# clawrim/gcn10

Hardware: AMD Instinct MI355X
Metric: CN Gpixels/sec (higher is better)
Workload: dtype u8

## Files before the change

### gcn10_amd/csrc/gcn10_context.hip

```cpp

#include <hip/hip_runtime.h>
#include <unistd.h>
#include <hip/hip_ext.h>

#include <cstdarg>
#include <cstdint>
#include <cstdio>
#include <cstring>
#include <new>

#include "gcn10_gpu.h"
#include "gcn10_device_util.hpp"
#include "gcn10_gpu_internal.hpp"
#include "gcn10_soil_readers.hpp"

using gcn10::as_stream;
using gcn10::fail;
using gcn10::kLut16Bytes;
using gcn10::kLut1Bytes;
using gcn10::use_device;

namespace gcn10 {

thread_local char g_err[512] = "";
// ... 430 lines not shown
            continue;
        ctx->opt.*o.field = value;
        if (o.field == &gcn10_gpu_ctx::Options::ilp1)
            ctx->opt.single.set = false;
        return GCN10_OK;
    }
    return fail(GCN10_E_INVAL, "gcn10_gpu_set_option: unknown option or bad value: %s=%d", name, value);
}

int gcn10_gpu_time_next_strip(gcn10_gpu_ctx *ctx, gcn10_event_t start, gcn10_event_t stop)
{
    if (!ctx || !start || !stop)
        return fail(GCN10_E_INVAL, "gcn10_gpu_time_next_strip: null argument");
    ctx->time_start = reinterpret_cast<hipEvent_t>(start);
    ctx->time_stop = reinterpret_cast<hipEvent_t>(stop);
    return GCN10_OK;
}

const char *gcn10_gpu_last_kernel_name(gcn10_gpu_ctx *ctx)
{
    return ctx ? ctx->last_kernel : "";
}

}
```

### gcn10_amd/csrc/gcn10_gpu_internal.hpp

```cpp
#ifndef GCN10_GPU_INTERNAL_HPP
#define GCN10_GPU_INTERNAL_HPP

#include <hip/hip_runtime.h>

#include <cstdint>

#include "gcn10_gpu.h"
#include "gcn10_strip_lanes.hpp"

namespace gcn10 {

int fail(int code, const char *fmt, ...) __attribute__((format(printf, 2, 3)));

#define HIP_TRY(expr)                                                                   \
    do {                                                                                \
        hipError_t e_ = (expr);                                                         \
        if (e_ != hipSuccess)                                                           \
            return gcn10::fail(e_ == hipErrorOutOfMemory ? GCN10_E_NOMEM : GCN10_E_HIP, \
                               "%s: %s", #expr, hipGetErrorString(e_));                 \
    } while (0)

int use_device(gcn10_gpu_ctx *ctx);
hipStream_t as_stream(gcn10_gpu_ctx *ctx, gcn10_stream_t s);
int grow_workspace(void **ws, size_t *cap, size_t need);
// ... 61 lines not shown

    struct SingleShape {
        bool set = false;
        int xcd_slabs = 1, grid_blocks_per_cu = 8, ilp = 2, prefetch = 1;
    };

    struct Options {
        int grid_blocks_per_cu = 16;
        int ilp16 = 0;
        int ilp1 = 2;
        int nontemporal = 1;
        int xcd_slabs = 1;
        int prefetch = 1;
        int compact_soil = 1;
        SingleShape single;
        int arena_segment_align = 4096;
        int deflate_wave_codes = 1;
        int fused_parse = 1;
        int fused_emit = 1;
        int event_sync_sleep_us = 0;
    } opt;

    const char *last_kernel = "";
    hipEvent_t time_start = nullptr, time_stop = nullptr;
    bool fused_ready = false;
    bool codes_ready = false;
    bool deflate_ready = false;

    struct Workspaces {
        void *deflate = nullptr;
        size_t deflate_cap = 0;
        void *inflate = nullptr;
        size_t inflate_cap = 0;
        void *lzw = nullptr;
        size_t lzw_cap = 0;
    } ws;
};

#endif
```

### gcn10_amd/csrc/gcn10_soil_readers.hpp

```cpp
#ifndef GCN10_SOIL_READERS_HPP
#define GCN10_SOIL_READERS_HPP

#include "gcn10_gpu_internal.hpp"

namespace gcn10 {

struct SoilView {
    const uint8_t *hx;
    const int32_t *cj;
    uint32_t stride, rows;

    __device__ __forceinline__ uint32_t clamp(uint32_t r) const { return r < rows ? r : rows - 1u; }
    __device__ __forceinline__ uint32_t row(uint32_t y) const { return clamp((uint32_t)cj[y]); }
    __device__ __forceinline__ const uint8_t *at(uint32_t r, uint32_t x) const { return hx + (size_t)r * stride + x; }
    __device__ __forceinline__ const uint8_t *ptr(uint32_t y, uint32_t x) const { return at(row(y), x); }
};

constexpr int kPlanes = 6;
constexpr int kLut16Plane = 256 * 16 + 16;
constexpr int kLut16Bytes = kPlanes * kLut16Plane;
constexpr int kPlane1 = 256 + 4;
constexpr int kLut1Bytes = kPlanes * kPlane1;

template <int THREADS>
__device__ __forceinline__ void stage_lut16(uint8_t *lds, const uint8_t *src)
{
    for (int i = threadIdx.x; i < kLut16Bytes / 16; i += THREADS)
        reinterpret_cast<u32x4 *>(lds)[i] = reinterpret_cast<const u32x4 *>(src)[i];
}

__device__ __forceinline__ const uint8_t *lut16_row(const uint8_t *lut, uint32_t plane, uint32_t lc)
{
    return lut + plane * (uint32_t)kLut16Plane + lc * 16u;
}

__device__ __forceinline__ uint32_t lut16_value(const uint8_t *lut, uint32_t plane, uint32_t lc, uint32_t k)
{
    return lut16_row(lut, plane, lc)[k];
}

__device__ __forceinline__ uint32_t perm(uint32_t hi, uint32_t lo, uint32_t sel)
{
    return __builtin_amdgcn_perm(hi, lo, sel);
}

__device__ __forceinline__ void transpose4x4(uint32_t a, uint32_t b, uint32_t c, uint32_t d, uint32_t &o0,
                                             uint32_t &o1, uint32_t &o2, uint32_t &o3)
{
    const uint32_t t0 = perm(b, a, 0x05010400u);
    const uint32_t t1 = perm(b, a, 0x07030602u);
    const uint32_t t2 = perm(d, c, 0x05010400u);
// ... 42 lines not shown
```

### gcn10_amd/csrc/gcn10_strip.hip

```cpp

#include <hip/hip_runtime.h>

#include <cstdint>
#include <cstdio>
#include <cstring>

#include "gcn10_gpu.h"
#include "gcn10_device_util.hpp"
#include "gcn10_gpu_internal.hpp"
#include "gcn10_soil_readers.hpp"

using gcn10::aligned16;
using gcn10::as_stream;
using gcn10::fail;
using gcn10::first_chunk;
using gcn10::kChunk;
using gcn10::kLut16Bytes;
using gcn10::kLut1Bytes;
using gcn10::kPlane1;
using gcn10::kPxPerLane;
using gcn10::kThreads;
using gcn10::launch_timed;
using gcn10::load16_aligned;
using gcn10::load16_aligned_nt;
using gcn10::load16_any;
using gcn10::popcount;
using gcn10::scalar_load_i32;
using gcn10::SoilView;
// ... 14 lines not shown
    uint32_t npix;
    uint32_t nvec16;
    uint32_t nchunks;
    uint32_t table_mask;
    uint32_t single_k;
    uint32_t xcd_slabs;
    const uint32_t *cx;
    const uint8_t *codes;
    uint32_t codes_stride;
    const uint32_t *soil_complex;
    uint32_t soil_gen;
};

enum { kLut16 = 0, kLut1 = 1 };
constexpr uint32_t kWavePx = 64u * kPxPerLane;
constexpr uint32_t kMinVectorW = kWavePx + 16u;

enum { kSoilBytes = 0, kSoilLanes = 1, kSoilPixels = 2 };

template <int ILP>
struct Trip {
    u32x4 e16[ILP], c16[ILP];
    uint32_t i0[ILP];
};

template <int ILP, bool NT>
__device__ __forceinline__ void issue_trip(const StripParams &p, uint32_t trip, uint32_t lane_off,
                                           uint32_t wave_off, Trip<ILP> &tr)
{
    uint32_t xb[ILP], r0[ILP], r1[ILP], wb[ILP];
#pragma unroll
    for (int u = 0; u < ILP; u++) {
        wb[u] = __builtin_amdgcn_readfirstlane((trip * ILP + u) * (uint32_t)kChunk + wave_off);
        const uint32_t wbc = wb[u] < p.npix ? wb[u] : 0u;
        const uint32_t y = wbc / p.W;
        xb[u] = wbc - y * p.W;
        r0[u] = (uint32_t)scalar_load_i32(p.soil.cj, y);
        r1[u] = (uint32_t)scalar_load_i32(p.soil.cj, y + 1u < p.rows ? y + 1u : y);
    }
#pragma unroll
    for (int u = 0; u < ILP; u++) {
        tr.i0[u] = wb[u] + lane_off;
        const uint8_t *pe = p.esa + (tr.i0[u] < p.nvec16 ? tr.i0[u] : 0u);
        tr.e16[u] = NT ? load16_aligned_nt(pe) : load16_aligned(pe);
    }
#pragma unroll
    for (int u = 0; u < ILP; u++) {
        uint32_t xl = xb[u] + lane_off;
        const bool wrap = xl >= p.W;
        xl = wrap ? xl - p.W : xl;
        const uint32_t row = p.soil.clamp(wrap ? r1[u] : r0[u]);
        const uint8_t *pa = p.soil.at(row, xl);
        u32x4 a = load16_any(pa);
        if (p.W & 15u) {
            const uint32_t n = p.W - xl;
            const bool strad = !wrap && n < (uint32_t)kPxPerLane;
            if (__builtin_amdgcn_ballot_w64(strad) != 0ull) {
                const uint8_t *pb = strad ? p.soil.at(p.soil.clamp(r1[u]), 0u) - n : pa;
                const u32x4 b = load16_any(pb);
                const uint32_t nn = strad ? n : (uint32_t)kPxPerLane;
#pragma unroll
                for (int j = 0; j < 4; j++) {
                    const int32_t m = (int32_t)nn - 4 * j;
                    const uint32_t mask = m >= 4 ? 0xffffffffu : (m <= 0 ? 0u : (1u << (8 * m)) - 1u);
                    a[j] = (a[j] & mask) | (b[j] & ~mask);
                }
// ... 40 lines not shown
    if (SOIL == kSoilLanes) {
        uint32_t cx[16];
#pragma unroll
        for (int j = 0; j < 4; j++) {
            const u32x4 c4 = *reinterpret_cast<const u32x4 *>(p.cx + ls.x + 4 * j);
#pragma unroll
            for (int q = 0; q < 4; q++)
                cx[4 * j + q] = c4[q];
        }
        ls.c_lo = cx[0];
        ls.c_hi = cx[15];
        uint32_t split = 0;
#pragma unroll
        for (int q = 0; q < 16; q++)
            split += cx[q] == ls.c_lo && split == (uint32_t)q ? 1u : 0u;
        ls.split = (int32_t)split;
#pragma unroll
        for (int j = 0; j < 4; j++)
            ls.mask[j] = split_mask(ls.split, j);
        ls.pair = __builtin_amdgcn_ballot_w64(ls.c_hi - ls.c_lo > 1u) == 0ull;
    }
}

template <int ILP, bool NT, int SOIL>
__device__ __forceinline__ void issue_lane_trip(const StripParams &p, const LaneSoil &ls, uint32_t trip,
                                                Trip<ILP> &tr)
{
    uint32_t o0[ILP], o1[ILP];
#pragma unroll
    for (int u = 0; u < ILP; u++) {
        const uint32_t y = ls.y_first + (trip * ILP + u) * ls.B;
        const uint32_t ya = y < p.rows ? y : p.rows - 1u;
        const uint32_t yb = y + 1u < p.rows ? y + 1u : p.rows - 1u;
        o0[u] = p.soil.clamp((uint32_t)scalar_load_i32(p.soil.cj, ya)) * p.codes_stride;
        o1[u] = p.soil.clamp((uint32_t)scalar_load_i32(p.soil.cj, yb)) * p.codes_stride;
    }
#pragma unroll
    for (int u = 0; u < ILP; u++) {
        const uint32_t i0 = ls.base + (trip * ILP + u) * ls.sub_px;
        const bool live = i0 < ls.lim;
        tr.i0[u] = live ? i0 : 0xffffffffu;
        const uint8_t *pe = p.esa + (live ? i0 : 0u);
        tr.e16[u] = NT ? load16_aligned_nt(pe) : load16_aligned(pe);
    }
#pragma unroll
    for (int u = 0; u < ILP; u++) {
        const uint32_t off = ls.wrap ? o1[u] : o0[u];
        if (SOIL == kSoilLanes) {
            typedef uint16_t u16_u __attribute__((aligned(1)));
            tr.c16[u][0] = *reinterpret_cast<const u16_u *>(p.codes + (off + ls.c_lo));
            if (!ls.pair)
                tr.c16[u][1] = p.codes[off + ls.c_hi];
        }
        else {
            const uint8_t *cr = p.codes + off;
            const u32x4 *pc = reinterpret_cast<const u32x4 *>(p.cx + ls.x);
            u32x4 a = { 0u, 0u, 0u, 0u };
#pragma unroll 1
            for (int j = 0; j < 4; j++) {
                const u32x4 c4 = pc[j];
                const uint32_t w = (uint32_t)cr[c4[0]] | (uint32_t)cr[c4[1]] << 8 | (uint32_t)cr[c4[2]] << 16 |
                                   (uint32_t)cr[c4[3]] << 24;
                a[0] = j == 0 ? w : a[0];
                a[1] = j == 1 ? w : a[1];
                a[2] = j == 2 ? w : a[2];
                a[3] = j == 3 ? w : a[3];
            }
            tr.c16[u] = a;
        }
    }
}

template <bool KEEP_MASKS>
__device__ __forceinline__ u32x4 mix_lane_codes(const LaneSoil &ls, const u32x4 &c)
{
    const uint32_t a = (c[0] & 0xffu) * 0x01010101u;
    const uint32_t b = (ls.pair ? (c[0] >> 8) & 0xffu : c[1] & 0xffu) * 0x01010101u;
    u32x4 cd;
    int32_t split = ls.split;
    if (!KEEP_MASKS)
        asm volatile("" : "+v"(split));
#pragma unroll
    for (int j = 0; j < 4; j++) {
        const uint32_t mask = KEEP_MASKS ? ls.mask[j] : split_mask(split, j);
        cd[j] = (a & mask) | (b & ~mask);
    }
    return cd;
}

template <int KIND, int COND_MASK, int ILP, bool NT, int SOIL>
__device__ __forceinline__ void finish_trip(const StripParams &p, const uint8_t *lut, uint32_t tmask,
                                            const Trip<ILP> &tr, const LaneSoil &ls)
{
#pragma unroll
    for (int u = 0; u < ILP; u++) {
        const bool live = tr.i0[u] < p.nvec16;
        const u32x4 c16 = SOIL == kSoilLanes ? mix_lane_codes<KIND == kLut1>(ls, tr.c16[u]) : tr.c16[u];
#pragma unroll
        for (int c = 0; c < 2; c++) {
            if (!(COND_MASK & (1 << c)))
                continue;
            if (KIND == kLut16) {
                uint32_t acc[9][4];
                gcn10::gather16(lut, tr.e16[u], c16, c, acc);
                if (live) {
#pragma unroll
                    for (int k = 0; k < 9; k++) {
                        if (tmask & (1u << k)) {
                            u32x4 v = {acc[k][0], acc[k][1], acc[k][2], acc[k][3]};
                            store16<NT>(p.out[c * 9 + k] + tr.i0[u], v);
                        }
                    }
                }
            }
            else {
                u32x4 v;
#pragma unroll
                for (int j = 0; j < 4; j++) {
                    const uint32_t e = tr.e16[u][j];
                    const uint32_t cd = c16[j];
                    uint32_t w = 0;
#pragma unroll
                    for (int q = 0; q < 4; q++) {
                        const uint32_t lc = (e >> (8 * q)) & 0xffu;
                        const uint32_t s = (cd >> (8 * q + 4 * c)) & 0xfu;
                        const uint32_t b = lut[s * (uint32_t)kPlane1 + lc];
                        w |= b << (8 * q);
                    }
                    v[j] = w;
                }
                if (live)
                    store16<NT>(p.out[c * 9 + p.single_k] + tr.i0[u], v);
            }
        }
    }
}

template <int KIND, int COND_MASK, int ILP, bool NT, bool PF, int SOIL>
__device__ __forceinline__ void strip_loop(const StripParams &p, const uint8_t *lut, uint32_t tmask)
{
    uint32_t step = 1u, end, trip = 0u, lane_off = 0u, wave_off = 0u;
    LaneSoil ls = {};
    if (SOIL == kSoilBytes) {
        lane_off = (threadIdx.x & 63u) * kPxPerLane;
        wave_off = __builtin_amdgcn_readfirstlane(threadIdx.x >> 6) * kWavePx;
        trip = first_chunk(p.nchunks, step, end, p.xcd_slabs != 0);
    }
    else {
        const gcn10::StripLanePlan pl = gcn10::strip_lane_plan(p.W, p.rows, gridDim.x, blockIdx.x, threadIdx.x,
                                                               p.xcd_slabs != 0, (uint32_t)ILP);
        end = __builtin_amdgcn_readfirstlane(pl.trips);
        if (!__builtin_amdgcn_readfirstlane((uint32_t)pl.active))
            return;
        lane_prologue<SOIL>(p, pl, ls);
    }
    if (trip >= end)
        return;
    auto issue = [&](uint32_t t, Trip<ILP> &tr) {
        if (SOIL == kSoilBytes)
            issue_trip<ILP, NT>(p, t, lane_off, wave_off, tr);
        else
            issue_lane_trip<ILP, NT, SOIL>(p, ls, t, tr);
    };
    if (!PF) {
        for (; trip < end; trip += step) {
            Trip<ILP> tr;
            issue(trip, tr);
            finish_trip<KIND, COND_MASK, ILP, NT, SOIL>(p, lut, tmask, tr, ls);
        }
    }
    else {
        Trip<ILP> ta, tb;
        issue(trip, ta);
        for (;;) {
            trip += step;
            if (trip >= end) {
                finish_trip<KIND, COND_MASK, ILP, NT, SOIL>(p, lut, tmask, ta, ls);
                break;
            }
            issue(trip, tb);
            finish_trip<KIND, COND_MASK, ILP, NT, SOIL>(p, lut, tmask, ta, ls);
            trip += step;
            if (trip >= end) {
                finish_trip<KIND, COND_MASK, ILP, NT, SOIL>(p, lut, tmask, tb, ls);
                break;
            }
            issue(trip, ta);
            finish_trip<KIND, COND_MASK, ILP, NT, SOIL>(p, lut, tmask, tb, ls);
        }
    }
}

template <int KIND, int COND_MASK, bool ALL_TABLES, int ILP, bool NT, bool PF>
__global__ __launch_bounds__(kThreads) void cn_strip_kernel(const StripParams p)
{
    constexpr int kLutBytes = KIND == kLut16 ? kLut16Bytes : kLut1Bytes;
    __shared__ __attribute__((aligned(16))) uint8_t lut[kLutBytes];

    if (KIND == kLut16) {
        gcn10::stage_lut16<kThreads>(lut, p.lut);
    }
    else {
        const uint32_t *src = reinterpret_cast<const uint32_t *>(p.lut);
        uint32_t *dst = reinterpret_cast<uint32_t *>(lut);
        for (int i = threadIdx.x; i < kLutBytes / 4; i += kThreads)
            dst[i] = src[i];
    }
    __syncthreads();

    const uint32_t tmask = ALL_TABLES ? 0x1ffu : p.table_mask;

    if (!p.codes)
        strip_loop<KIND, COND_MASK, ILP, NT, PF, kSoilBytes>(p, lut, tmask);
    else if ((uint32_t)scalar_load_i32(reinterpret_cast<const int32_t *>(p.soil_complex), 0u) != p.soil_gen)
        strip_loop<KIND, COND_MASK, ILP, NT, PF, kSoilLanes>(p, lut, tmask);
    else
        strip_loop<KIND, COND_MASK, ILP, NT, PF, kSoilPixels>(p, lut, tmask);

    if (blockIdx.x == 0 && threadIdx.x < p.npix - p.nvec16) {
        const uint32_t i = p.nvec16 + threadIdx.x;
        const uint32_t y = i / p.W;
        const uint32_t x = i - y * p.W;
        const uint32_t lc = p.esa[i];
        const uint32_t cd = *p.soil.ptr(y, x);
#pragma unroll
        for (int c = 0; c < 2; c++) {
            if (!(COND_MASK & (1 << c)))
                continue;
            const uint32_t s = (cd >> (4 * c)) & 0xfu;
            if (KIND == kLut16) {
                const uint8_t *row = gcn10::lut16_row(lut, s, lc);
                for (int k = 0; k < 9; k++)
                    if (tmask & (1u << k))
                        p.out[c * 9 + k][i] = row[k];
            }
            else {
                p.out[c * 9 + p.single_k][i] = lut[s * (uint32_t)kPlane1 + lc];
            }
        }
    }
// ... 146 lines not shown
    const uint32_t grid = stream_grid(ctx, p.nchunks, tuned ? ctx->opt.single.grid_blocks_per_cu : 0);
    if (tuned)
        p.xcd_slabs = (uint32_t)ctx->opt.single.xcd_slabs;
    if (all_aligned && ctx->opt.compact_soil && (p.W & 15u) == 0u &&
        gcn10::strip_lane_plan(p.W, p.rows, grid, 0u, 0u, p.xcd_slabs != 0, (uint32_t)ilp).B > 0u) {
        p.soil = SoilView{ nullptr, cj, ctx->tile.hx_stride, ctx->tile.hx_rows };
        p.cx = ctx->tile.d_cx;
        p.codes = ctx->tile.d_codes;
        p.codes_stride = ctx->tile.codes_stride;
        p.soil_complex = ctx->tile.d_soil_complex;
        p.soil_gen = ctx->tile.soil_gen;
    }
    else {
        rc = gcn10::bind_soil(ctx, who, W, s, cj, &p.soil);
        if (rc)
            return rc;
    }
    if (!all_aligned) {
        p.lut = ctx->d_lut16;
        const uint32_t g = stream_grid(ctx, ((uint64_t)p.npix + kThreads - 1) / kThreads);
        void *args[] = { &p, &cond_mask };
        HIP_TRY(launch_timed(ctx, reinterpret_cast<const void *>(cn_strip_bytes), g, args, s));
        ctx->last_kernel = "cn_strip_bytes";
    }
    else {
        if (single) {
            p.single_k = (uint32_t)__builtin_ctz(table_mask);
            p.lut = ctx->d_lut1 + (size_t)p.single_k * kLut1Bytes;
        }
        else {
            p.lut = ctx->d_lut16;
        }
        const StripKernel *k = find_strip_kernel(single, cond_mask, table_mask == 0x1ffu, ilp, ctx->opt.nontemporal != 0,
                                                 (tuned ? ctx->opt.single.prefetch : ctx->opt.prefetch) != 0);
        if (!k)
            return fail(GCN10_E_INVAL, "gcn10_gpu_cn_strip: no kernel for ilp=%d", ilp);
        void *args[] = { &p };
        HIP_TRY(launch_timed(ctx, reinterpret_cast<const void *>(k->fn), grid, args, s));
        ctx->last_kernel = k->name;
    }
    HIP_TRY(hipGetLastError());
    return GCN10_OK;
}

size_t gcn10_gpu_strip_algorithmic_bytes(int W, int rows, int hsx, int hsy, unsigned cond_mask,
                                         unsigned table_mask)
{
    if (W <= 0 || rows <= 0)
        return 0;
    const size_t n_out = (size_t)popcount(cond_mask & 3u) * (size_t)popcount(table_mask & 0x1ffu);
    return (size_t)W * rows * (1 + n_out) + (size_t)(hsx > 0 ? hsx : 0) * (hsy > 0 ? hsy : 0) +
           4 * ((size_t)W + rows);
}

int gcn10_gpu_stream_copy(gcn10_gpu_ctx *ctx, const void *src, void *dst, size_t bytes, gcn10_stream_t stream)
{
    int rc = use_device(ctx);
    if (rc)
        return rc;
    if (bytes == 0)
        return GCN10_OK;
    if (!src || !dst || (bytes & 15u) || !aligned16(src) || !aligned16(dst) || bytes / 16 > 0x7fffffffull)
// ... 104 lines not shown
```

### gcn10_amd/gpu.py

```python
from __future__ import annotations

import ctypes as C
import os
from typing import Optional, Sequence

import numpy as np

from . import host as _host

_HERE = os.path.dirname(os.path.abspath(__file__))
LIB_PATH = os.environ.get("GCN10_GPU_LIB") or os.path.join(_HERE, "libgcn10_gpu.so")
_lib = None

N_TABLES = 9
N_RASTERS = 18
COND_DRAINED = 1
COND_UNDRAINED = 2
ALL_TABLES = 0x1FF
NODATA = 255

ABI_SYMBOLS = (
    "gcn10_gpu_abi_version", "gcn10_gpu_device_count", "gcn10_gpu_init", "gcn10_gpu_destroy",
    "gcn10_gpu_last_error", "gcn10_gpu_device_info", "gcn10_gpu_malloc", "gcn10_gpu_free",
    "gcn10_gpu_host_alloc", "gcn10_gpu_host_free", "gcn10_gpu_memcpy_h2d",
    "gcn10_gpu_memcpy_d2h", "gcn10_gpu_memset", "gcn10_gpu_stream_create",
    "gcn10_gpu_stream_destroy", "gcn10_gpu_stream_sync", "gcn10_gpu_device_sync",
    "gcn10_gpu_event_create", "gcn10_gpu_event_destroy", "gcn10_gpu_event_record",
    "gcn10_gpu_event_sync", "gcn10_gpu_stream_wait_event", "gcn10_gpu_event_elapsed_ms",
    "gcn10_gpu_set_tables", "gcn10_gpu_resample", "gcn10_gpu_modify_hysogs_data",
    "gcn10_gpu_calculate_cn", "gcn10_gpu_prepare_tile", "gcn10_gpu_cn_strip",
    "gcn10_gpu_strip_algorithmic_bytes", "gcn10_gpu_last_kernel_name", "gcn10_gpu_set_option",
    "gcn10_gpu_deflate_arena_bound", "gcn10_gpu_deflate_strip", "gcn10_gpu_time_next_strip",
    "gcn10_gpu_pci_bus_id", "gcn10_gpu_deflate_fused_strip",
    "gcn10_gpu_deflate_fused_available",
    "gcn10_gpu_inflate_tiles", "gcn10_gpu_stream_copy", "gcn10_gpu_tune_single_raster",
    "gcn10_gpu_soil_words_state", "gcn10_gpu_lzw_arena_bound", "gcn10_gpu_lzw_strip",
    "gcn10_gpu_inflate_codecs", "gcn10_gpu_overview_nearest", "gcn10_gpu_overview_average",
    "gcn10_gpu_pair_histogram_codes", "gcn10_gpu_pair_histogram",
    "gcn10_gpu_verify_strip", "gcn10_gpu_verify_buffers", "gcn10_gpu_zonal_pair_histogram",
    "gcn10_gpu_aggregate", "gcn10_gpu_grid_sums", "gcn10_gpu_grid_finish",
    "gcn10_gpu_set_weights", "gcn10_gpu_grid_sums_weighted", "gcn10_gpu_grid_finish_weighted",
)


def pair_histogram_codes() -> np.ndarray:
    codes = np.zeros(PAIR_HIST_BINS, np.uint8)
    n = lib().gcn10_gpu_pair_histogram_codes(codes.ctypes.data_as(C.POINTER(C.c_uint8)))
    if n != PAIR_HIST_BINS:
        raise RuntimeError("gcn10_gpu_pair_histogram_codes returned %d" % n)
    return codes


TILE_RAW, TILE_PREDICTOR2, TILE_LZW = 1, 2, 4
CODEC_DEFLATE, CODEC_RAW, CODEC_LZW = 1, 2, 4
# ... 32 lines not shown
            "gcn10_gpu_host_alloc": (i, [vp, sz, C.POINTER(vp)]),
            "gcn10_gpu_host_free": (i, [vp, vp]),
            "gcn10_gpu_memcpy_h2d": (i, [vp, vp, vp, sz, vp]),
            "gcn10_gpu_memcpy_d2h": (i, [vp, vp, vp, sz, vp]),
            "gcn10_gpu_memset": (i, [vp, vp, i, sz, vp]),
            "gcn10_gpu_stream_create": (i, [vp, C.POINTER(vp)]),
            "gcn10_gpu_stream_destroy": (i, [vp, vp]),
            "gcn10_gpu_stream_sync": (i, [vp, vp]),
            "gcn10_gpu_device_sync": (i, [vp]),
            "gcn10_gpu_event_create": (i, [vp, C.POINTER(vp)]),
            "gcn10_gpu_event_destroy": (i, [vp, vp]),
            "gcn10_gpu_event_record": (i, [vp, vp, vp]),
            "gcn10_gpu_event_sync": (i, [vp, vp]),
            "gcn10_gpu_stream_wait_event": (i, [vp, vp, vp]),
            "gcn10_gpu_event_elapsed_ms": (i, [vp, vp, vp, C.POINTER(C.c_float)]),
            "gcn10_gpu_set_tables": (i, [vp, vp, i]),
            "gcn10_gpu_resample": (i, [vp, vp, i, i, vp, vp, i, i, vp, vp]),
            "gcn10_gpu_modify_hysogs_data": (i, [vp, vp, sz, i, vp]),
            "gcn10_gpu_calculate_cn": (i, [vp, vp, vp, sz, i, vp, vp]),
            "gcn10_gpu_prepare_tile": (i, [vp, vp, i, i, vp, i, vp]),
            "gcn10_gpu_cn_strip": (i, [vp, vp, i, i, vp, u, u, C.POINTER(vp), vp]),
            "gcn10_gpu_strip_algorithmic_bytes": (sz, [i, i, i, i, u, u]),
            "gcn10_gpu_last_kernel_name": (C.c_char_p, [vp]),
            "gcn10_gpu_set_option": (i, [vp, C.c_char_p, i]),
            "gcn10_gpu_time_next_strip": (i, [vp, vp, vp]),
            "gcn10_gpu_stream_copy": (i, [vp, vp, vp, sz, vp]),
            "gcn10_gpu_tune_single_raster": (i, [vp, vp, i, i, vp, u, u, vp, sz, sz, C.POINTER(vp),
                                                 C.POINTER(C.c_float), C.c_char_p, sz, vp]),
            "gcn10_gpu_pci_bus_id": (i, [i, C.c_char_p, sz]),
            "gcn10_gpu_soil_words_state": (i, [vp, vp]),
            "gcn10_gpu_deflate_fused_strip": (i, [vp, vp, i, i, vp, u, u, vp, sz, vp, vp, vp]),
            "gcn10_gpu_deflate_fused_available": (i, [vp]),
            "gcn10_gpu_inflate_tiles": (i, [vp, vp, vp, i, u, vp, sz, vp, vp]),
            "gcn10_gpu_inflate_codecs": (i, []),
            "gcn10_gpu_deflate_arena_bound": (sz, [i, i, i]),
            "gcn10_gpu_deflate_strip": (i, [vp, vp, i, i, i, vp, sz, vp, vp, vp]),
            "gcn10_gpu_lzw_arena_bound": (sz, [i, i, i]),
            "gcn10_gpu_lzw_strip": (i, [vp, vp, i, i, i, vp, sz, vp, vp, vp]),
            "gcn10_gpu_overview_nearest": (i, [vp, vp, i, i, i, vp, vp]),
            "gcn10_gpu_overview_average": (i, [vp, vp, i, i, i, i, vp, u, u, i, C.POINTER(vp), vp]),
            "gcn10_gpu_pair_histogram_codes": (i, [C.POINTER(C.c_uint8)]),
            "gcn10_gpu_pair_histogram": (i, [vp, vp, i, i, vp, vp, vp]),
            "gcn10_gpu_verify_strip": (i, [vp, vp, i, i, vp, C.c_uint, C.c_uint, vp, sz, i, vp, vp]),
            "gcn10_gpu_verify_buffers": (i, [vp, vp, sz, vp, sz, i, i, i, C.c_uint, vp, vp]),
            "gcn10_gpu_zonal_pair_histogram": (i, [vp, vp, i, i, vp, vp, vp, sz, i, vp, vp]),
            "gcn10_gpu_aggregate": (i, [vp, vp, i, i, vp, i, i, i, u, u, C.POINTER(vp), sz, vp]),
            "gcn10_gpu_grid_sums": (i, [vp, vp, i, i, vp, vp, vp, i, i, u, u, vp, vp]),
            "gcn10_gpu_grid_finish": (i, [vp, vp, i, sz, vp, vp, C.c_uint32, vp, vp]),
            "gcn10_gpu_set_weights": (i, [vp, vp]),
            "gcn10_gpu_grid_sums_weighted": (i, [vp, vp, i, i, vp, vp, vp, i, i, u, u, vp, vp]),
            "gcn10_gpu_grid_finish_weighted": (i, [vp, vp, i, sz, vp, vp, vp, C.c_uint32, vp, vp]),
        }
        for name, (res, args) in sig.items():
            fn = getattr(L, name)
            fn.restype = res
            fn.argtypes = args
        _lib = L
    return _lib


def device_count() -> int:
    return int(lib().gcn10_gpu_device_count())


def strip_algorithmic_bytes(W: int, rows: int, hsx: int, hsy: int, cond_mask: int,
                            table_mask: int) -> int:
    return int(lib().gcn10_gpu_strip_algorithmic_bytes(W, rows, hsx, hsy, cond_mask, table_mask))


class DevBuf:

    def __init__(self, eng: "Engine", nbytes: int):
        self.eng = eng
        self.nbytes = int(nbytes)
        p = C.c_void_p()
        eng._chk(lib().gcn10_gpu_malloc(eng._ctx, self.nbytes, C.byref(p)), "gcn10_gpu_malloc")
# ... 133 lines not shown

    def tune_single_raster(self, esa, W: int, rows: int, cj, cond_mask: int, table_mask: int, arena, arena_bytes: int,
                           step: int = 16 << 20, stream=None):
        import json as _json
        best = C.c_void_p()
        ms = C.c_float()
        rep = C.create_string_buffer(512)
        self._chk(lib().gcn10_gpu_tune_single_raster(self._ctx, esa, W, rows, cj, cond_mask, table_mask, arena,
                                                     int(arena_bytes), int(step), C.byref(best), C.byref(ms), rep, 512,
                                                     stream), "gcn10_gpu_tune_single_raster")
        return best.value, float(ms.value), _json.loads(rep.value.decode() or "{}")

    def stream_copy(self, src, dst, nbytes: int, stream=None):
        self._chk(lib().gcn10_gpu_stream_copy(self._ctx, src, dst, int(nbytes), stream), "gcn10_gpu_stream_copy")

    def soil_words_state(self, stream=None) -> int:
        rc = lib().gcn10_gpu_soil_words_state(self._ctx, stream)
        if rc < 0:
            self._chk(rc, "gcn10_gpu_soil_words_state")
        return rc

    def last_kernel_name(self) -> str:
        return lib().gcn10_gpu_last_kernel_name(self._ctx).decode()

    def set_tables(self, tables: np.ndarray):
        t = np.ascontiguousarray(tables, dtype=np.int32)
        if t.ndim == 2:
            t = t[None]
        if t.ndim != 3 or t.shape[1:] != (256, 5):
            raise ValueError("tables must be int32[n,256,5]")
        self._chk(lib().gcn10_gpu_set_tables(self._ctx, t.ctypes.data, t.shape[0]),
                  "gcn10_gpu_set_tables")
        self.n_tables = t.shape[0]

    def resample(self, coarse_d: int, hsx: int, hsy: int, ci_d: int, cj_d: int, W: int,
                 rows: int, out_d: int, stream=None):
        self._chk(lib().gcn10_gpu_resample(self._ctx, coarse_d, hsx, hsy, ci_d, cj_d, W, rows,
                                           out_d, stream), "gcn10_gpu_resample")

    def modify_hysogs_data(self, h_d: int, npix: int, drained: bool, stream=None):
        self._chk(lib().gcn10_gpu_modify_hysogs_data(self._ctx, h_d, npix, int(bool(drained)),
                                                     stream), "gcn10_gpu_modify_hysogs_data")

    def calculate_cn(self, esa_d: int, hsg_d: int, npix: int, table_index: int, out_d: int,
                     stream=None):
        self._chk(lib().gcn10_gpu_calculate_cn(self._ctx, esa_d, hsg_d, npix, table_index, out_d,
# ... 250 lines not shown
```

### include/gcn10_gpu.h

```cpp
#ifndef GCN10_GPU_H
#define GCN10_GPU_H

#include <stddef.h>
#include <stdint.h>

#ifdef __cplusplus
extern "C" {
#endif

#define GCN10_GPU_ABI_VERSION 3

enum {
    GCN10_OK = 0,
    GCN10_E_INVAL = -1,
    GCN10_E_HIP = -2,
    GCN10_E_NOMEM = -3,
    GCN10_E_STATE = -4,
    GCN10_E_NODEVICE = -5
};

#define GCN10_N_TABLES 9
#define GCN10_N_CONDS 2
#define GCN10_N_RASTERS 18
#define GCN10_COND_DRAINED 1u
// ... 162 lines not shown
                           const uint8_t *const got[GCN10_N_RASTERS], size_t got_stride, int y0,
                           gcn10_verify_count *counts_dev, gcn10_stream_t stream);
int gcn10_gpu_verify_buffers(gcn10_gpu_ctx *ctx, const uint8_t *const want[GCN10_N_RASTERS], size_t want_stride,
                             const uint8_t *const got[GCN10_N_RASTERS], size_t got_stride, int W, int rows, int y0,
                             unsigned raster_mask, gcn10_verify_count *counts_dev, gcn10_stream_t stream);

int gcn10_gpu_set_option(gcn10_gpu_ctx *ctx, const char *name, int value);

int gcn10_gpu_time_next_strip(gcn10_gpu_ctx *ctx, gcn10_event_t start, gcn10_event_t stop);

int gcn10_gpu_stream_copy(gcn10_gpu_ctx *ctx, const void *src, void *dst, size_t bytes,
                          gcn10_stream_t stream);

int gcn10_gpu_tune_single_raster(gcn10_gpu_ctx *ctx, const uint8_t *esa, int W, int rows,
                                 const int32_t *cj, unsigned cond_mask, unsigned table_mask,
                                 uint8_t *arena, size_t arena_bytes, size_t step,
                                 uint8_t **best_out, float *best_ms, char *report, size_t report_cap,
                                 gcn10_stream_t stream);

int gcn10_gpu_soil_words_state(gcn10_gpu_ctx *ctx, gcn10_stream_t stream);

const char *gcn10_gpu_last_kernel_name(gcn10_gpu_ctx *ctx);

#ifdef __cplusplus
}
#endif
#endif
```

Baseline: 3020.

## Split strip loop into unchecked full trips and a bounds-checked tail

Specializes the strip kernel's main loop with a FULL template flag so interior trips skip per-element bounds clamps and live checks, leaving only the final trip checked. It restructures the prefetch double-buffer loop, hoists the output pointers into scalar registers, makes the pair/non-pair soil-lane choice a compile-time branch, and rewrites LUT staging as an unrolled load-then-store. Sched barriers around the stores pin the instruction order. A plan-reporting API and profiling scripts are also added. The extra template variants grow code size and register pressure.

Measured after the change: 3041, median of 6. About the same (+0.7%).

```diff
diff --git a/gcn10_amd/csrc/gcn10_context.hip b/gcn10_amd/csrc/gcn10_context.hip
--- a/gcn10_amd/csrc/gcn10_context.hip
+++ b/gcn10_amd/csrc/gcn10_context.hip
@@ -476,4 +476,12 @@
     return ctx ? ctx->last_kernel : "";
 }
 
-}
+int gcn10_gpu_last_strip_plan(gcn10_gpu_ctx *ctx, int out[4])
+{
+    if (!ctx || !out)
+        return fail(GCN10_E_INVAL, "gcn10_gpu_last_strip_plan: null argument");
+    memcpy(out, ctx->last_plan, sizeof ctx->last_plan);
+    return GCN10_OK;
+}
+
+}
diff --git a/gcn10_amd/csrc/gcn10_gpu_internal.hpp b/gcn10_amd/csrc/gcn10_gpu_internal.hpp
--- a/gcn10_amd/csrc/gcn10_gpu_internal.hpp
+++ b/gcn10_amd/csrc/gcn10_gpu_internal.hpp
@@ -107,6 +107,7 @@
     } opt;
 
     const char *last_kernel = "";
+    int last_plan[4] = { 0, 0, 0, 0 };
     hipEvent_t time_start = nullptr, time_stop = nullptr;
     bool fused_ready = false;
     bool codes_ready = false;
diff --git a/gcn10_amd/csrc/gcn10_soil_readers.hpp b/gcn10_amd/csrc/gcn10_soil_readers.hpp
--- a/gcn10_amd/csrc/gcn10_soil_readers.hpp
+++ b/gcn10_amd/csrc/gcn10_soil_readers.hpp
@@ -22,11 +22,24 @@
 constexpr int kPlane1 = 256 + 4;
 constexpr int kLut1Bytes = kPlanes * kPlane1;
 
+template <int THREADS, int N, typename T>
+__device__ __forceinline__ void stage_table(T *lds, const T *src)
+{
+    static_assert(N >= THREADS, "a table of at least one item per thread");
+    constexpr int kSteps = (N + THREADS - 1) / THREADS;
+    T v[kSteps];
+#pragma unroll
+    for (int k = 0; k < kSteps; k++)
+        v[k] = src[(int)threadIdx.x + ((k + 1) * THREADS <= N ? k * THREADS : N - THREADS)];
+#pragma unroll
+    for (int k = 0; k < kSteps; k++)
+        lds[(int)threadIdx.x + ((k + 1) * THREADS <= N ? k * THREADS : N - THREADS)] = v[k];
+}
+
 template <int THREADS>
 __device__ __forceinline__ void stage_lut16(uint8_t *lds, const uint8_t *src)
 {
-    for (int i = threadIdx.x; i < kLut16Bytes / 16; i += THREADS)
-        reinterpret_cast<u32x4 *>(lds)[i] = reinterpret_cast<const u32x4 *>(src)[i];
+    stage_table<THREADS, kLut16Bytes / 16>(reinterpret_cast<u32x4 *>(lds), reinterpret_cast<const u32x4 *>(src));
 }
 
 __device__ __forceinline__ const uint8_t *lut16_row(const uint8_t *lut, uint32_t plane, uint32_t lc)
diff --git a/gcn10_amd/csrc/gcn10_strip.hip b/gcn10_amd/csrc/gcn10_strip.hip
--- a/gcn10_amd/csrc/gcn10_strip.hip
+++ b/gcn10_amd/csrc/gcn10_strip.hip
@@ -4,6 +4,7 @@
 #include <cstdint>
 #include <cstdio>
 #include <cstring>
+#include <type_traits>
 
 #include "gcn10_gpu.h"
 #include "gcn10_device_util.hpp"
@@ -64,9 +65,11 @@
 struct Trip {
     u32x4 e16[ILP], c16[ILP];
     uint32_t i0[ILP];
+    uint16_t lo[ILP];
+    uint8_t hi[ILP];
 };
 
-template <int ILP, bool NT>
+template <int ILP, bool NT, bool FULL>
 __device__ __forceinline__ void issue_trip(const StripParams &p, uint32_t trip, uint32_t lane_off,
                                            uint32_t wave_off, Trip<ILP> &tr)
 {
@@ -74,7 +77,7 @@
 #pragma unroll
     for (int u = 0; u < ILP; u++) {
         wb[u] = __builtin_amdgcn_readfirstlane((trip * ILP + u) * (uint32_t)kChunk + wave_off);
-        const uint32_t wbc = wb[u] < p.npix ? wb[u] : 0u;
+        const uint32_t wbc = FULL || wb[u] < p.npix ? wb[u] : 0u;
         const uint32_t y = wbc / p.W;
         xb[u] = wbc - y * p.W;
         r0[u] = (uint32_t)scalar_load_i32(p.soil.cj, y);
@@ -83,7 +86,7 @@
 #pragma unroll
     for (int u = 0; u < ILP; u++) {
         tr.i0[u] = wb[u] + lane_off;
-        const uint8_t *pe = p.esa + (tr.i0[u] < p.nvec16 ? tr.i0[u] : 0u);
+        const uint8_t *pe = p.esa + (FULL || tr.i0[u] < p.nvec16 ? tr.i0[u] : 0u);
         tr.e16[u] = NT ? load16_aligned_nt(pe) : load16_aligned(pe);
     }
 #pragma unroll
@@ -170,7 +173,7 @@
     }
 }
 
-template <int ILP, bool NT, int SOIL>
+template <int ILP, bool NT, int SOIL, bool FULL, bool PAIR>
 __device__ __forceinline__ void issue_lane_trip(const StripParams &p, const LaneSoil &ls, uint32_t trip,
                                                 Trip<ILP> &tr)
 {
@@ -178,15 +181,15 @@
 #pragma unroll
     for (int u = 0; u < ILP; u++) {
         const uint32_t y = ls.y_first + (trip * ILP + u) * ls.B;
-        const uint32_t ya = y < p.rows ? y : p.rows - 1u;
-        const uint32_t yb = y + 1u < p.rows ? y + 1u : p.rows - 1u;
+        const uint32_t ya = FULL || y < p.rows ? y : p.rows - 1u;
+        const uint32_t yb = FULL || y + 1u < p.rows ? y + 1u : p.rows - 1u;
         o0[u] = p.soil.clamp((uint32_t)scalar_load_i32(p.soil.cj, ya)) * p.codes_stride;
         o1[u] = p.soil.clamp((uint32_t)scalar_load_i32(p.soil.cj, yb)) * p.codes_stride;
     }
 #pragma unroll
     for (int u = 0; u < ILP; u++) {
         const uint32_t i0 = ls.base + (trip * ILP + u) * ls.sub_px;
-        const bool live = i0 < ls.lim;
+        const bool live = FULL || i0 < ls.lim;
         tr.i0[u] = live ? i0 : 0xffffffffu;
         const uint8_t *pe = p.esa + (live ? i0 : 0u);
         tr.e16[u] = NT ? load16_aligned_nt(pe) : load16_aligned(pe);
@@ -196,9 +199,9 @@
         const uint32_t off = ls.wrap ? o1[u] : o0[u];
         if (SOIL == kSoilLanes) {
             typedef uint16_t u16_u __attribute__((aligned(1)));
-            tr.c16[u][0] = *reinterpret_cast<const u16_u *>(p.codes + (off + ls.c_lo));
-            if (!ls.pair)
-                tr.c16[u][1] = p.codes[off + ls.c_hi];
+            tr.lo[u] = *reinterpret_cast<const u16_u *>(p.codes + (off + ls.c_lo));
+            if (!PAIR)
+                tr.hi[u] = p.codes[off + ls.c_hi];
         }
         else {
             const uint8_t *cr = p.codes + off;
@@ -219,11 +222,11 @@
     }
 }
 
-template <bool KEEP_MASKS>
-__device__ __forceinline__ u32x4 mix_lane_codes(const LaneSoil &ls, const u32x4 &c)
-{
-    const uint32_t a = (c[0] & 0xffu) * 0x01010101u;
-    const uint32_t b = (ls.pair ? (c[0] >> 8) & 0xffu : c[1] & 0xffu) * 0x01010101u;
+template <bool KEEP_MASKS, bool PAIR>
+__device__ __forceinline__ u32x4 mix_lane_codes(const LaneSoil &ls, uint16_t lo, uint8_t hi)
+{
+    const uint32_t a = (lo & 0xffu) * 0x01010101u;
+    const uint32_t b = (PAIR ? (uint32_t)lo >> 8 : (uint32_t)hi) * 0x01010101u;
     u32x4 cd;
     int32_t split = ls.split;
     if (!KEEP_MASKS)
@@ -236,14 +239,48 @@
     return cd;
 }
 
-template <int KIND, int COND_MASK, int ILP, bool NT, int SOIL>
-__device__ __forceinline__ void finish_trip(const StripParams &p, const uint8_t *lut, uint32_t tmask,
-                                            const Trip<ILP> &tr, const LaneSoil &ls)
+typedef __attribute__((address_space(1))) uint8_t *global_u8_t;
+typedef __attribute__((address_space(1))) u32x4 *global_u32x4_t;
+
+template <int KIND>
+struct StripOuts {
+    global_u8_t r[KIND == kLut16 ? GCN10_N_RASTERS : 2];
+};
+
+template <bool NT>
+__device__ __forceinline__ void store16_global(global_u8_t p, u32x4 v)
+{
+    if (NT)
+        __builtin_nontemporal_store(v, (global_u32x4_t)p);
+    else
+        *(global_u32x4_t)p = v;
+}
+
+template <int KIND, int COND_MASK>
+__device__ __forceinline__ StripOuts<KIND> strip_outs(const StripParams &p)
+{
+    StripOuts<KIND> o;
+#pragma unroll
+    for (int i = 0; i < (int)(sizeof o.r / sizeof o.r[0]); i++) {
+        const int c = KIND == kLut16 ? i / 9 : i;
+        global_u8_t ptr = nullptr;
+        if (COND_MASK & (1 << c)) {
+            ptr = (global_u8_t)(KIND == kLut16 ? p.out[i] : p.out[c * 9 + p.single_k]);
+            asm volatile("" : "+s"(ptr));
+        }
+        o.r[i] = ptr;
+    }
+    return o;
+}
+
+template <int KIND, int COND_MASK, int ILP, bool NT, int SOIL, bool FULL, bool PAIR>
+__device__ __forceinline__ void finish_trip(const StripParams &p, const StripOuts<KIND> &o, const uint8_t *lut,
+                                            uint32_t tmask, const Trip<ILP> &tr, const LaneSoil &ls)
 {
 #pragma unroll
     for (int u = 0; u < ILP; u++) {
-        const bool live = tr.i0[u] < p.nvec16;
-        const u32x4 c16 = SOIL == kSoilLanes ? mix_lane_codes<KIND == kLut1>(ls, tr.c16[u]) : tr.c16[u];
+        const bool live = FULL || tr.i0[u] < p.nvec16;
+        const u32x4 c16 = SOIL == kSoilLanes ? mix_lane_codes<KIND == kLut1, PAIR>(ls, tr.lo[u], tr.hi[u]) : tr.c16[u];
 #pragma unroll
         for (int c = 0; c < 2; c++) {
             if (!(COND_MASK & (1 << c)))
@@ -251,15 +288,19 @@
             if (KIND == kLut16) {
                 uint32_t acc[9][4];
                 gcn10::gather16(lut, tr.e16[u], c16, c, acc);
+                if (FULL)
+                    __builtin_amdgcn_sched_barrier(0);
                 if (live) {
 #pragma unroll
                     for (int k = 0; k < 9; k++) {
                         if (tmask & (1u << k)) {
                             u32x4 v = {acc[k][0], acc[k][1], acc[k][2], acc[k][3]};
-                            store16<NT>(p.out[c * 9 + k] + tr.i0[u], v);
+                            store16_global<NT>(o.r[c * 9 + k] + tr.i0[u], v);
                         }
                     }
                 }
+                if (FULL)
+                    __builtin_amdgcn_sched_barrier(0);
             }
             else {
                 u32x4 v;
@@ -277,22 +318,30 @@
                     }
                     v[j] = w;
                 }
+                if (FULL)
+                    __builtin_amdgcn_sched_barrier(0);
                 if (live)
-                    store16<NT>(p.out[c * 9 + p.single_k] + tr.i0[u], v);
+                    store16_global<NT>(o.r[c] + tr.i0[u], v);
+                if (FULL)
+                    __builtin_amdgcn_sched_barrier(0);
             }
         }
     }
 }
 
 template <int KIND, int COND_MASK, int ILP, bool NT, bool PF, int SOIL>
-__device__ __forceinline__ void strip_loop(const StripParams &p, const uint8_t *lut, uint32_t tmask)
-{
-    uint32_t step = 1u, end, trip = 0u, lane_off = 0u, wave_off = 0u;
+__device__ __forceinline__ void strip_loop(const StripParams &p, const StripOuts<KIND> &o, const uint8_t *lut,
+                                           uint32_t tmask)
+{
+    uint32_t step = 1u, end, full_end, trip = 0u, lane_off = 0u, wave_off = 0u;
     LaneSoil ls = {};
+    bool has_group = true;
     if (SOIL == kSoilBytes) {
         lane_off = (threadIdx.x & 63u) * kPxPerLane;
         wave_off = __builtin_amdgcn_readfirstlane(threadIdx.x >> 6) * kWavePx;
         trip = first_chunk(p.nchunks, step, end, p.xcd_slabs != 0);
+        full_end = p.nvec16 / (uint32_t)(kChunk * ILP);
+        full_end = full_end < end ? full_end : end;
     }
     else {
         const gcn10::StripLanePlan pl = gcn10::strip_lane_plan(p.W, p.rows, gridDim.x, blockIdx.x, threadIdx.x,
@@ -301,42 +350,85 @@
         if (!__builtin_amdgcn_readfirstlane((uint32_t)pl.active))
             return;
         lane_prologue<SOIL>(p, pl, ls);
-    }
-    if (trip >= end)
+        full_end = end > 0u ? end - 1u : 0u;
+        has_group = pl.active;
+    }
+    if (trip >= end || !has_group)
         return;
-    auto issue = [&](uint32_t t, Trip<ILP> &tr) {
+    auto run = [&](auto pair_tag) {
+    constexpr bool PAIR = decltype(pair_tag)::value;
+    auto issue_full = [&](uint32_t t, Trip<ILP> &tr) {
         if (SOIL == kSoilBytes)
-            issue_trip<ILP, NT>(p, t, lane_off, wave_off, tr);
+            issue_trip<ILP, NT, true>(p, t, lane_off, wave_off, tr);
         else
-            issue_lane_trip<ILP, NT, SOIL>(p, ls, t, tr);
+            issue_lane_trip<ILP, NT, SOIL, true, PAIR>(p, ls, t, tr);
+    };
+    auto issue_last = [&](uint32_t t, Trip<ILP> &tr) {
+        if (SOIL == kSoilBytes)
+            issue_trip<ILP, NT, false>(p, t, lane_off, wave_off, tr);
+        else
+            issue_lane_trip<ILP, NT, SOIL, false, PAIR>(p, ls, t, tr);
+    };
+    auto finish_full = [&](const Trip<ILP> &tr) {
+        finish_trip<KIND, COND_MASK, ILP, NT, SOIL, true, PAIR>(p, o, lut, tmask, tr, ls);
+    };
+    auto finish_last = [&](const Trip<ILP> &tr) {
+        finish_trip<KIND, COND_MASK, ILP, NT, SOIL, false, PAIR>(p, o, lut, tmask, tr, ls);
     };
     if (!PF) {
+        for (; trip < full_end; trip += step) {
+            Trip<ILP> tr;
+            issue_full(trip, tr);
+            finish_full(tr);
+        }
         for (; trip < end; trip += step) {
             Trip<ILP> tr;
-            issue(trip, tr);
-            finish_trip<KIND, COND_MASK, ILP, NT, SOIL>(p, lut, tmask, tr, ls);
+            issue_last(trip, tr);
+            finish_last(tr);
+        }
+    }
+    else if (trip >= full_end) {
+        for (; trip < end; trip += step) {
+            Trip<ILP> tr;
+            issue_last(trip, tr);
+            finish_last(tr);
         }
     }
     else {
         Trip<ILP> ta, tb;
-        issue(trip, ta);
-        for (;;) {
+        auto hand_over = [&](const Trip<ILP> &cur, Trip<ILP> &other) {
+            const bool more = trip < end;
+            if (more)
+                issue_last(trip, other);
+            finish_full(cur);
+            if (more)
+                finish_last(other);
+        };
+        const uint32_t n_full = (full_end - trip + step - 1u) / step;
+        issue_full(trip, ta);
+        trip += step;
+        for (uint32_t pair = (n_full - 1u) / 2u; pair > 0u; pair--) {
+            issue_full(trip, tb);
+            finish_full(ta);
+            issue_full(trip + step, ta);
+            finish_full(tb);
+            trip += 2u * step;
+        }
+        if (n_full & 1u) {
+            hand_over(ta, tb);
+        }
+        else {
+            issue_full(trip, tb);
+            finish_full(ta);
             trip += step;
-            if (trip >= end) {
-                finish_trip<KIND, COND_MASK, ILP, NT, SOIL>(p, lut, tmask, ta, ls);
-                break;
-            }
-            issue(trip, tb);
-            finish_trip<KIND, COND_MASK, ILP, NT, SOIL>(p, lut, tmask, ta, ls);
-            trip += step;
-            if (trip >= end) {
-                finish_trip<KIND, COND_MASK, ILP, NT, SOIL>(p, lut, tmask, tb, ls);
-                break;
-            }
-            issue(trip, ta);
-            finish_trip<KIND, COND_MASK, ILP, NT, SOIL>(p, lut, tmask, tb, ls);
-        }
-    }
+            hand_over(tb, ta);
+        }
+    }
+    };
+    if (SOIL != kSoilLanes || ls.pair)
+        run(std::true_type{});
+    else
+        run(std::false_type{});
 }
 
 template <int KIND, int COND_MASK, bool ALL_TABLES, int ILP, bool NT, bool PF>
@@ -349,21 +441,20 @@
         gcn10::stage_lut16<kThreads>(lut, p.lut);
     }
     else {
-        const uint32_t *src = reinterpret_cast<const uint32_t *>(p.lut);
-        uint32_t *dst = reinterpret_cast<uint32_t *>(lut);
-        for (int i = threadIdx.x; i < kLutBytes / 4; i += kThreads)
-            dst[i] = src[i];
+        gcn10::stage_table<kThreads, kLutBytes / 4>(reinterpret_cast<uint32_t *>(lut),
+                                                    reinterpret_cast<const uint32_t *>(p.lut));
     }
     __syncthreads();
 
     const uint32_t tmask = ALL_TABLES ? 0x1ffu : p.table_mask;
+    const StripOuts<KIND> o = strip_outs<KIND, COND_MASK>(p);
 
     if (!p.codes)
-        strip_loop<KIND, COND_MASK, ILP, NT, PF, kSoilBytes>(p, lut, tmask);
+        strip_loop<KIND, COND_MASK, ILP, NT, PF, kSoilBytes>(p, o, lut, tmask);
     else if ((uint32_t)scalar_load_i32(reinterpret_cast<const int32_t *>(p.soil_complex), 0u) != p.soil_gen)
-        strip_loop<KIND, COND_MASK, ILP, NT, PF, kSoilLanes>(p, lut, tmask);
+        strip_loop<KIND, COND_MASK, ILP, NT, PF, kSoilLanes>(p, o, lut, tmask);
     else
-        strip_loop<KIND, COND_MASK, ILP, NT, PF, kSoilPixels>(p, lut, tmask);
+        strip_loop<KIND, COND_MASK, ILP, NT, PF, kSoilPixels>(p, o, lut, tmask);
 
     if (blockIdx.x == 0 && threadIdx.x < p.npix - p.nvec16) {
         const uint32_t i = p.nvec16 + threadIdx.x;
@@ -556,6 +647,8 @@
         void *args[] = { &p, &cond_mask };
         HIP_TRY(launch_timed(ctx, reinterpret_cast<const void *>(cn_strip_bytes), g, args, s));
         ctx->last_kernel = "cn_strip_bytes";
+        const int plan[4] = { (int)g, 1, 0, 0 };
+        memcpy(ctx->last_plan, plan, sizeof plan);
     }
     else {
         if (single) {
@@ -572,6 +665,16 @@
         void *args[] = { &p };
         HIP_TRY(launch_timed(ctx, reinterpret_cast<const void *>(k->fn), grid, args, s));
         ctx->last_kernel = k->name;
+        if (p.codes) {
+            const gcn10::StripLanePlan pl = gcn10::strip_lane_plan(p.W, p.rows, grid, 0u, 0u, p.xcd_slabs != 0,
+                                                                   (uint32_t)ilp);
+            const int plan[4] = { (int)grid, (int)pl.pieces, (int)pl.B, (int)pl.trips };
+            memcpy(ctx->last_plan, plan, sizeof plan);
+        }
+        else {
+            const int plan[4] = { (int)grid, p.xcd_slabs && grid % 8u == 0u && p.nchunks >= grid ? 8 : 1, 0, 0 };
+            memcpy(ctx->last_plan, plan, sizeof plan);
+        }
     }
     HIP_TRY(hipGetLastError());
     return GCN10_OK;
diff --git a/gcn10_amd/gpu.py b/gcn10_amd/gpu.py
--- a/gcn10_amd/gpu.py
+++ b/gcn10_amd/gpu.py
@@ -29,7 +29,8 @@
     "gcn10_gpu_event_sync", "gcn10_gpu_stream_wait_event", "gcn10_gpu_event_elapsed_ms",
     "gcn10_gpu_set_tables", "gcn10_gpu_resample", "gcn10_gpu_modify_hysogs_data",
     "gcn10_gpu_calculate_cn", "gcn10_gpu_prepare_tile", "gcn10_gpu_cn_strip",
-    "gcn10_gpu_strip_algorithmic_bytes", "gcn10_gpu_last_kernel_name", "gcn10_gpu_set_option",
+    "gcn10_gpu_strip_algorithmic_bytes", "gcn10_gpu_last_kernel_name", "gcn10_gpu_last_strip_plan",
+    "gcn10_gpu_set_option",
     "gcn10_gpu_deflate_arena_bound", "gcn10_gpu_deflate_strip", "gcn10_gpu_time_next_strip",
     "gcn10_gpu_pci_bus_id", "gcn10_gpu_deflate_fused_strip",
     "gcn10_gpu_deflate_fused_available",
@@ -108,6 +109,7 @@
             "gcn10_gpu_cn_strip": (i, [vp, vp, i, i, vp, u, u, C.POINTER(vp), vp]),
             "gcn10_gpu_strip_algorithmic_bytes": (sz, [i, i, i, i, u, u]),
             "gcn10_gpu_last_kernel_name": (C.c_char_p, [vp]),
+            "gcn10_gpu_last_strip_plan": (i, [vp, C.POINTER(i * 4)]),
             "gcn10_gpu_set_option": (i, [vp, C.c_char_p, i]),
             "gcn10_gpu_time_next_strip": (i, [vp, vp, vp]),
             "gcn10_gpu_stream_copy": (i, [vp, vp, vp, sz, vp]),
@@ -138,6 +140,8 @@
             "gcn10_gpu_grid_finish_weighted": (i, [vp, vp, i, sz, vp, vp, vp, C.c_uint32, vp, vp]),
         }
         for name, (res, args) in sig.items():
+            if name == "gcn10_gpu_last_strip_plan" and not hasattr(L, name):
+                continue
             fn = getattr(L, name)
             fn.restype = res
             fn.argtypes = args
@@ -317,6 +321,11 @@
 
     def last_kernel_name(self) -> str:
         return lib().gcn10_gpu_last_kernel_name(self._ctx).decode()
+
+    def last_strip_plan(self):
+        out = (C.c_int * 4)()
+        self._chk(lib().gcn10_gpu_last_strip_plan(self._ctx, C.byref(out)), "gcn10_gpu_last_strip_plan")
+        return tuple(int(v) for v in out)
 
     def set_tables(self, tables: np.ndarray):
         t = np.ascontiguousarray(tables, dtype=np.int32)
diff --git a/include/gcn10_gpu.h b/include/gcn10_gpu.h
--- a/include/gcn10_gpu.h
+++ b/include/gcn10_gpu.h
@@ -208,6 +208,8 @@
 
 const char *gcn10_gpu_last_kernel_name(gcn10_gpu_ctx *ctx);
 
+int gcn10_gpu_last_strip_plan(gcn10_gpu_ctx *ctx, int out[4]);
+
 #ifdef __cplusplus
 }
 #endif
diff --git a/profiles/strip_full_trips/grid_ab.py b/profiles/strip_full_trips/grid_ab.py
--- /dev/null
+++ b/profiles/strip_full_trips/grid_ab.py
@@ -0,0 +1,59 @@
+#!/usr/bin/env python3
+import json
+import os
+import sys
+
+import numpy as np
+
+ROOT = os.path.dirname(os.path.dirname(os.path.dirname(os.path.abspath(__file__))))
+sys.path.insert(0, ROOT)
+import bench
+from gcn10_amd import gpu, host
+
+
+def main():
+    grids = [int(a) for a in sys.argv[1].split(",")]
+    rounds = int(sys.argv[2]) if len(sys.argv) > 2 else 5
+    n = int(sys.argv[3]) if len(sys.argv) > 3 else 10
+    size = int(os.environ.get("AB_SIZE", "36000"))
+    eng = gpu.Engine(0)
+    eng.set_tables(host.load_all_lookup_tables(os.path.join(ROOT, "tests", "golden", "lookups")))
+    esa, gt, coarse, soil_gt = bench.synth_block(1, size, "iid")
+    hs = coarse.shape[0]
+    ci, cj = host.build_index_maps(gt, soil_gt, size, size, hs, hs)
+    d_esa, d_coarse, d_ci, d_cj = eng.upload(esa), eng.upload(coarse), eng.upload(ci), eng.upload(cj)
+    outs = [eng.alloc(size * size) for _ in range(18)]
+    ptrs = [b.ptr for b in outs]
+    eng.prepare_tile(d_coarse.ptr, hs, hs, d_ci.ptr, size)
+    ev = [(eng.event_create(), eng.event_create()) for _ in range(n)]
+    res = {g: [] for g in grids}
+    plan = {}
+    for r in range(rounds):
+        for g in grids:
+            eng.set_option("defaults", 0)
+            if g > 0:
+                eng.set_option("grid_blocks_per_cu", g)
+            for _ in range(2):
+                eng.cn_strip(d_esa.ptr, size, size, d_cj.ptr, 3, 0x1FF, ptrs)
+            eng.sync()
+            for i in range(n):
+                eng.time_next_strip(ev[i][0], ev[i][1])
+                eng.cn_strip(d_esa.ptr, size, size, d_cj.ptr, 3, 0x1FF, ptrs)
+            eng.sync()
+            ms = [eng.elapsed_ms(a, b) for a, b in ev]
+            if hasattr(eng, "last_strip_plan"):
+                plan[g] = eng.last_strip_plan()
+            res[g].append(float(np.mean(ms)))
+            print(json.dumps({"round": r, "grid_blocks_per_cu": g, "kernel": eng.last_kernel_name(),
+                              "avg_ms": round(float(np.mean(ms)), 4), "min_ms": round(float(np.min(ms)), 4),
+                              "max_ms": round(float(np.max(ms)), 4), "plan": plan.get(g)}), flush=True)
+    for g in grids:
+        v = res[g]
+        print(json.dumps({"summary": g, "median_of_rounds": round(float(np.median(v)), 4), "min": round(min(v), 4),
+                          "max": round(max(v), 4), "range": round(max(v) - min(v), 4)}), flush=True)
+    chk = eng.download(ptrs[0], (64, size))
+    print(json.dumps({"lib": gpu.LIB_PATH, "raster0_rows64_sum": int(chk.astype(np.int64).sum())}))
+
+
+if __name__ == "__main__":
+    main()
diff --git a/profiles/strip_full_trips/loop_waits.py b/profiles/strip_full_trips/loop_waits.py
--- /dev/null
+++ b/profiles/strip_full_trips/loop_waits.py
@@ -0,0 +1,64 @@
+#!/usr/bin/env python3
+import re
+import subprocess
+import sys
+
+KERNELS = ("<0, 3, true, 1, true, true>", "<1, 1, true, 2, true, false>", "<1, 1, true, 1, true, false>",
+           "<1, 1, true, 2, true, true>", "<1, 1, true, 4, true, false>")
+
+
+def event(ins):
+    op = ins.split()[0]
+    if op.startswith("global_load"):
+        return "L"
+    if op.startswith("global_store"):
+        return "S"
+    if op.startswith("ds_write"):
+        return "D"
+    if op.startswith("s_load"):
+        return "K"
+    if op in ("s_cbranch_execz", "s_cbranch_execnz"):
+        return "X"
+    if op == "s_waitcnt":
+        m = re.search(r"vmcnt\((\d+)\)", ins)
+        return "w" + m.group(1) if m else None
+    return None
+
+
+def main(path):
+    lines = open(path, errors="replace").read().split("\n")
+    syms = [l.split()[1] for l in lines if l.strip().startswith(".amdhsa_kernel ")]
+    nice = subprocess.run(["c++filt"], input="\n".join(syms), capture_output=True, text=True).stdout.split("\n")
+    for sym, name in zip(syms, nice):
+        if "cn_strip_kernel" not in name or not any(k in name for k in KERNELS):
+            continue
+        start = next(i for i, l in enumerate(lines) if l.startswith(sym + ":"))
+        end = next(i for i in range(start, len(lines)) if lines[i].startswith(".Lfunc_end"))
+        body = lines[start:end]
+        print("== cn_strip_kernel%s" % name[name.index("<"):name.index(">") + 1])
+        bar = next(i for i, l in enumerate(body) if l.strip().startswith("s_barrier"))
+        ev = [e for e in (event(l.strip()) for l in body[:bar] if l.startswith("\t")) if e and e != "K"]
+        print("   staging: " + " ".join(ev))
+        labels = [i for i, l in enumerate(body) if re.match(r"\.LBB\d+_\d+:", l)] + [len(body)]
+        n_loop = 0
+        for a, i in enumerate(labels[:-1]):
+            m = re.match(r"(\.LBB\d+_\d+):.*Inner Loop Header", body[i])
+            if not m:
+                continue
+            head = m.group(1)[2:]
+            mine = [(x, labels[b + 1]) for b, x in enumerate(labels[:-1])
+                    if x == i or re.search(r"in Loop: Header=%s\b" % head, body[x])]
+            mine = [r for r in mine if r[0] >= i] + [r for r in mine if r[0] < i]
+            ins = [l.strip() for x, y in mine for l in body[x + 1:y] if l.startswith("\t")]
+            ev = [(event(l), l) for l in ins]
+            ev = [(e, l) for e, l in ev if e]
+            if any(e in ("L", "S") for e, _ in ev):
+                n_loop += 1
+                print("   loop %d (%s, %d instructions): %s" % (n_loop, head, len(ins), " ".join(e for e, _ in ev)))
+                for e, l in ev:
+                    if e[0] in "wXK":
+                        print("        " + re.sub(r"\s+", " ", l))
+
+
+if __name__ == "__main__":
+    main(sys.argv[1])
diff --git a/profiles/strip_full_trips/summarize.py b/profiles/strip_full_trips/summarize.py
--- /dev/null
+++ b/profiles/strip_full_trips/summarize.py
@@ -0,0 +1,37 @@
+#!/usr/bin/env python3
+import glob
+import json
+import os
+import statistics
+import sys
+
+FIELDS = {"config4": (("roofline", "avg_launch_ms"), ("value", None)),
+          "default": (("also", "avg_launch_ms"), ("roofline", "avg_launch_ms"), ("ms_per_step", None))}
+
+
+def line(path):
+    for text in open(path):
+        if text.lstrip().startswith("{"):
+            return json.loads(text)
+    raise ValueError(path)
+
+
+def main(d):
+    for what, fields in FIELDS.items():
+        runs = {b: [line(p) for p in sorted(glob.glob(os.path.join(d, "bench_%s_%s_*.json" % (what, b))))]
+                for b in ("parent", "new")}
+        for top, sub in fields:
+            for b in ("parent", "new"):
+                v = [r[top] if sub is None else r[top][sub] for r in runs[b]]
+                print("%-8s %-24s %-6s median %.4f  min %.4f  max %.4f  range %.4f  %s" % (
+                    what, top + ("." + sub if sub else ""), b, statistics.median(v), min(v), max(v), max(v) - min(v), v))
+        for b in ("parent", "new"):
+            checks = [r.get("self_check") for r in runs[b] if r.get("self_check")]
+            if checks:
+                print("%-8s self-check %-6s %d runs, differing pixels %s; kernels %s" % (
+                    what, b, len(checks), [c.get("differing") for c in checks],
+                    sorted({r["roofline"].get("kernel", "?") for r in runs[b]})))
+
+
+if __name__ == "__main__":
+    main(sys.argv[1] if len(sys.argv) > 1 else os.path.dirname(os.path.abspath(__file__)))
```
